# fulcrumgenomics/fgumi

Hardware: AMD Instinct MI355X
Metric: simplex consensus throughput, input raw reads/s (depth-8 x 150bp) (higher is better)
Workload: dtype f64

## Files before the change

fgumi_amd/csrc/api.cpp:

```cpp
#include <chrono>
#include <cstdio>
#include <stdexcept>
#include <cstring>
#include <mutex>
#include <map>
#include <mutex>
#include <string>
#include <thread>
#include "engine.h"
#include <gnu/libc-version.h>
#include <cmath>
#include "fastpath.h"
#include "host_common.h"
#include "simgen.h"
#include "canon_core.h"
#include "reject_core.h"
#include "aln_tags_core.h"

namespace fgx {
using canon::CANON_KIND_DUPLEX; using canon::CANON_KIND_CODEC; using canon::CANON_KIND_SIMPLEX;
uint32_t launch_canon_molecules(hipStream_t s, int kind, const canon::Params& P, const canon::CodecParams& PC, const uint8_t* d_blob,
                                const uint64_t* d_rec_off, const uint32_t* d_rec_len, const uint32_t* d_grp_first, const uint32_t* d_def, uint32_t nd,
                                const uint64_t* d_first, uint8_t* d_out, const uint64_t* d_out_off, uint32_t* d_out_len, int* d_status,
                                canon::Delta* d_delta, DevBuf& slabs, canon::RefRuns* d_runs, const rej::Params* PS);
// ... 1357 lines not shown
uint32_t fgx_debug_last_duplex_deep(const fgx_caller* c) { return (c && c->fast) ? c->fast->fp.last_duplex_deep : 0u; }
uint32_t fgx_debug_last_duplex_deep_capped(const fgx_caller* c) { return (c && c->fast) ? c->fast->fp.last_duplex_deep_capped : 0u; }
uint32_t fgx_debug_last_codec_deep(const fgx_caller* c) { return (c && c->fast) ? c->fast->fp.last_codec_deep : 0u; }
uint32_t fgx_debug_last_codec_deep_capped(const fgx_caller* c) { return (c && c->fast) ? c->fast->fp.last_codec_deep_capped : 0u; }
uint32_t fgx_debug_last_boundary_rounds(const fgx_caller* c) { return c ? c->last_boundary_rounds : 0u; }
void fgx_debug_last_split_builds(const fgx_caller* c, uint64_t* out4) {
  if (!out4) return;
  out4[0] = out4[1] = out4[2] = out4[3] = 0;
  if (c && c->fast) { const FastPath& f = c->fast->fp; out4[0] = f.last_packed_families; out4[1] = f.last_classic_families; out4[2] = f.last_split_build; out4[3] = f.last_first_stage_retries; }
}
void fgx_debug_split_first_slice(double mean_records, int packed, uint32_t* out4) {
  if (!out4) return;
  out4[0] = s2_first_slice_bytes(mean_records, packed != 0);
  out4[1] = out4[0] - s2_tile_bytes(mean_records);
  out4[2] = (uint32_t)sizeof(FullItem);
  out4[3] = S2_FLAG_DESC_BYTES;
}
void fgx_debug_last_packed_rows(const fgx_caller* c, uint64_t* out2) {
  if (!out2) return;
  out2[0] = out2[1] = 0;
  if (c && c->fast) { out2[0] = c->fast->fp.last_packed_clean; out2[1] = c->fast->fp.last_packed_general; }
}
void fgx_debug_last_packed_overlap(const fgx_caller* c, uint64_t* out3) {
  if (!out3) return;
  for (int i = 0; i < 3; i++) out3[i] = (c && c->fast) ? c->fast->fp.last_packed_overlap[i] : 0;
}
void fgx_debug_last_full_results(const fgx_caller* c, uint64_t* out4) {
  if (!out4) return;
  for (int i = 0; i < 4; i++) out4[i] = (c && c->fast) ? c->fast->fp.last_full_results[i] : 0;
}
uint64_t fgx_debug_last_full_results_over(const fgx_caller* c) { return (c && c->fast) ? c->fast->fp.last_full_results[4] : 0; }
int fgx_debug_full_range_whole(uint32_t base, uint32_t items, uint32_t cap) { return full_range_whole(base, items, cap) ? 1 : 0; }
void fgx_debug_last_chain(const fgx_caller* c, uint32_t* out2) { if (out2) { out2[0] = (c && c->fast) ? c->fast->fp.last_launches : 0u; out2[1] = (c && c->fast) ? c->fast->fp.last_host_syncs : 0u; } }
uint32_t fgx_debug_last_routed(const fgx_caller* c) { return (c && c->fast) ? c->fast->fp.last_routed : 0u; }
int fgx_debug_last_direct(const fgx_caller* c) { return (c && c->fast) ? c->fast->fp.last_direct : 0; }
void fgx_set_general_only(fgx_caller* c, int on) { if (c) c->general_only = on != 0; }
void fgx_set_fast_lds_bytes(fgx_caller* c, uint32_t bytes) { if (c) { if (!c->fast) c->fast = new FastState(); c->fast->fp.lds_tile_bytes_large = bytes; } }

int fgx_call_columns(fgx_caller* c, const uint8_t* bases, const uint8_t* quals, uint32_t n_cols, uint32_t depth, uint8_t* out_base,
                     uint8_t* out_qual, uint32_t* out_depth, uint32_t* out_errors) {
  if (!c) return 1;
  c->err.clear();
  try {
    ColumnBatch& B = c->batch;
    B.clear();
    std::vector<uint8_t> rb, rq;
    for (uint32_t j0 = 0; j0 < n_cols; j0 += 4096) {
      uint32_t w = std::min<uint32_t>(4096, n_cols - j0);
      uint32_t rd0 = (uint32_t)B.reads.size();
      for (uint32_t i = 0; i < depth; i++) {
        rb.resize(w); rq.resize(w);
        for (uint32_t k = 0; k < w; k++) { rb[k] = bases[(size_t)(j0 + k) * depth + i]; rq[k] = quals[(size_t)(j0 + k) * depth + i]; }
        B.add_read(rb.data(), rq.data(), w);
      }
      if (depth == 0) { B.add_job(rd0, 0, w); continue; }
      if (depth == 1) { rb.assign(w, 'N'); rq.assign(w, 0); B.add_read(rb.data(), rq.data(), w); B.add_job(rd0, 2, w); }
      else B.add_job(rd0, depth, w);
    }
    ColParams prm{0, 0};
    c->run_columns(B, prm);
    for (uint32_t j = 0; j < n_cols; j++) { out_base[j] = B.ob[j]; out_qual[j] = B.oq[j]; out_depth[j] = B.od[j]; out_errors[j] = B.oe[j]; }
    return 0;
  } catch (const std::exception& ex) { c->err = ex.what(); return 3; }
}

int fgx_device_libm(fgx_caller* c, int op, const double* x, double* y, uint64_t n) {
// ... 118 lines not shown
```

fgumi_amd/csrc/fastpath.hip:

```cpp
#if !defined(FGX_WAVEMU)
#include <hipcub/hipcub.hpp>
#endif
#include "bamrec.h"
#include "canon_core.h"
#include "engine.h"
#include <cstdlib>
#include <memory>
#include <string>
#include <type_traits>
#include "fastpath.h"
#include "gate_core.h"
#include "packed_core.h"
#include "record_core.h"

#if defined(FGX_WAVEMU)
#define FGX_DYN_LDS(name) uint8_t* const name = wavemu::dyn_lds()
#define FGX_PIN(...) ((void)0)
#define FGX_UNDEF4(a, b, c, d) do { a = 0; b = 0; c = 0; d = 0; } while (0)
#define FGX_MEM_PIN() ((void)0)
#define FGX_CONST_AS
#else
#define FGX_DYN_LDS(name) extern __shared__ __align__(16) uint8_t name[]
#define FGX_PIN(...) asm volatile("" : __VA_ARGS__)
#define FGX_UNDEF4(a, b, c, d) asm volatile("" : "=v"(a), "=v"(b), "=v"(c), "=v"(d))
// ... 2487 lines not shown
    const double ll[4] = {sLL[k][0], sLL[k][1], sLL[k][2], sLL[k][3]};
    const uint32_t ob = sObs[k];
    const bool is_rx = (dest >> 63) != 0;
    const ConsensusTables& T = is_rx ? P.TU->t : P.T->t;
    int bi;
    uint8_t q;
    call_full(T, ll, &bi, &q);
    if (is_rx) {
      const uint64_t d = dest & ~(1ull << 63);
      P.rx_base[(size_t)(d >> 8) * P.rx_stride + (d & 0xFF)] = bi >= 0 ? "ACGT"[bi] : 'N';
    } else finish(dest, bi, q, ob & 0xFF, (ob >> 8) & 0xFF, (ob >> 16) & 0xFF, ob >> 24, (sKind[k] >> 31) != 0, sSlot[k]);
  }
  if (P.stats) {
    const uint32_t t_arr = wave_sum(n_arr), t_scat = wave_sum(n_scat);
    if ((threadIdx.x & 63) == 0) {
      unsigned long long* fs = P.stats + (size_t)((blockIdx.x * 4 + blockIdx.y + (threadIdx.x >> 6)) & (STAT_SLOTS - 1)) * FULL_STATS_STRIDE;
      if (t_arr) atomicAdd(&fs[0], (unsigned long long)t_arr);
      if (t_scat) atomicAdd(&fs[1], (unsigned long long)t_scat);
    }
  }
}

#include "record_writers.inc"

#include "simplex_wave2.inc"
#include "simplex_seg.inc"
#include "simplex_split.inc"
#include "simplex_deep.inc"
#include "duplex_deep.inc"
#include "codec_deep.inc"
#include "simplex_wide.inc"
#include "duplex_meth.inc"

__global__ void k_col_bound(const uint32_t* __restrict__ grp_first, const uint32_t* __restrict__ rec_len, const uint64_t* __restrict__ rec_off, uint32_t n_grp,
                            uint64_t* __restrict__ bound, uint32_t max_ends, uint4* __restrict__ fam_desc, unsigned long long* __restrict__ small_recs, uint64_t* __restrict__ sizes_tail) {
  uint32_t g = blockIdx.x * blockDim.x + threadIdx.x;
  {
    uint32_t mine = 0;
    if (g < n_grp) { const uint32_t n = grp_first[g + 1] - grp_first[g]; mine = (grp_first[g + 1] >= grp_first[g] && n <= 64u) ? n : 0u; }
    __shared__ unsigned int s_tot;
    if (threadIdx.x == 0) s_tot = 0;
    __syncthreads();
    const uint32_t tot = wave_sum(mine);
    if ((threadIdx.x & 63) == 0 && tot) atomicAdd(&s_tot, tot);
    __syncthreads();
    if (threadIdx.x == 0 && s_tot) atomicAdd(small_recs, (unsigned long long)s_tot);
  }
  if (g >= n_grp) return;
  if (g == n_grp - 1) { bound[n_grp] = 0; *sizes_tail = 0; }
  uint32_t a = grp_first[g], b = grp_first[g + 1], mx = 0;
  {
    uint32_t r = a;
    if (((uintptr_t)rec_len & 15u) == 0) {
      for (; r < b && (r & 3u); r++) { const uint32_t l = rec_len[r]; mx = l > mx ? l : mx; }
      for (; r + 4 <= b; r += 4) {
        const uint4 v = *(const uint4*)(rec_len + r);
        const uint32_t m01 = v.x > v.y ? v.x : v.y, m23 = v.z > v.w ? v.z : v.w, m4 = m01 > m23 ? m01 : m23;
        mx = m4 > mx ? m4 : mx;
      }
    }
    for (; r < b; r++) { const uint32_t l = rec_len[r]; mx = l > mx ? l : mx; }
  }
  uint32_t lb = mx > 33 ? (mx - 33) * 2 / 3 + 1 : 1;
  uint32_t ends = (b - a) < max_ends ? (b - a) : max_ends;
  bound[g] = (uint64_t)ends * lb + COL_BOUND_PAD;
  uint64_t lo = 0;
  uint32_t span = 0xFFFFFFFFu;
  if (b > a) {
    lo = rec_off[a];
    const uint64_t hi = rec_off[b - 1] + rec_len[b - 1];
    if (hi >= lo && hi - lo < 0xFFFFFFFFull) span = (uint32_t)(hi - lo);
  }
  fam_desc[g] = make_uint4((uint32_t)lo, (uint32_t)(lo >> 32), span, b - a);
}

__global__ void k_reduce_stats(const unsigned long long* __restrict__ slots, unsigned long long* __restrict__ out, const unsigned long long* __restrict__ full_stats, uint32_t full_out) {
  uint32_t k = threadIdx.x;
  if (k >= 32 && k < 32 + FULL_STATS_N + OV_STATS_N) {
    unsigned long long v = 0;
    for (int i = 0; i < STAT_SLOTS; i++) v += full_stats[(size_t)i * FULL_STATS_STRIDE + (k - 32)];
    out[full_out + (k - 32)] = v;
  }
  if (k >= 32) return;
  unsigned long long v = 0;
  for (int i = 0; i < STAT_SLOTS; i++) v += slots[(size_t)i * 32 + k];
  out[k < FGX_STATS_LEN ? k : 40 + (k - FGX_STATS_LEN)] = v;
}

}

#define FGX_SYNC(st) do { fp.last_host_syncs++; hip_check(hipStreamSynchronize(st), "sync"); } while (0)
#define FGX_LAUNCH(kernel, grid, block, lds, st, ...) do { fp.last_launches++; hipLaunchKernelGGL((kernel), grid, block, lds, st, __VA_ARGS__); hip_check(hipGetLastError(), #kernel " launch"); } while (0)

void FastPath::release() {
  for (DevBuf* b : {&d_ends, &d_sizes, &d_offsets, &d_code, &d_qual, &d_depth, &d_err, &d_misc, &d_deferred, &d_out, &d_scan_tmp, &d_strings, &d_obs, &d_obs_all, &d_retry2,
                    &d_retry, &d_bound, &d_colbase, &d_statslots, &d_full_items, &d_full_count, &d_full_res, &d_full_flag, &d_retry_old, &d_w2img, &d_famdesc, &d_fwimg,
                    &d_split_rec, &d_split_fam, &d_split_out, &d_route, &d_s2img, &d_dir_size, &d_dir_off, &d_dir_base, &d_slot_desc, &d_slot_err, &d_out2, &d_scan_tmp2, &d_big, &d_deep_sizes, &d_deep_row0, &d_deep_rows, &d_deep_walk, &d_deep_fams, &d_deep_out, &d_deep_out2, &d_wide_scratch, &d_wide_pass, &d_wide_pass0, &d_wide_depth, &d_mflag, &d_mu, &d_mt, &d_mslot, &d_mcontigs})
    b->free_();
  for (int i = 0; i < 4; i++) if (ev[i]) { (void)hipEventDestroy(ev[i]); ev[i] = nullptr; }
  if (s2) {
    (void)hipStreamDestroy(s2); s2 = nullptr;
    for (int i = 0; i < MAX_CHUNKS; i++) { if (ev_chunk[i]) { (void)hipEventDestroy(ev_chunk[i]); ev_chunk[i] = nullptr; } if (ev_cols[i]) { (void)hipEventDestroy(ev_cols[i]); ev_cols[i] = nullptr; } }
    if (ev_fin) { (void)hipEventDestroy(ev_fin); ev_fin = nullptr; }
    if (ev_sample) { (void)hipEventDestroy(ev_sample); ev_sample = nullptr; }
  }
}
// ... 172 lines not shown
  void next_list(uint32_t n) { cur_list = lists[out_list]; n_cur = n; out_list ^= 1; }

  void set_up() {
    fp.last_meth_device = 0; fp.last_meth_clipped = 0; fp.last_direct = 0; fp.last_split_chunks = 0;
    if (!fp.canon_second_pass) fp.last_deep_clipped = fp.last_duplex_deep = fp.last_duplex_deep_capped = fp.last_codec_deep = fp.last_codec_deep_capped = 0;
    fp.last_routed = 0; fp.last_big_families = 0; fp.last_deep_families = 0; fp.last_wide_families = 0; fp.last_packed_families = 0; fp.last_classic_families = 0; fp.last_packed_clean = 0; fp.last_packed_general = 0; for (uint64_t& v : fp.last_packed_overlap) v = 0; for (uint64_t& v : fp.last_full_results) v = 0; fp.last_split_build = 0; fp.last_first_stage_retries = 0;
    fp.d_ends.reserve((size_t)n_slots * (duplex ? sizeof(DuplexDesc) : codec ? sizeof(CodecDesc) : sizeof(EndDesc)));
    fp.d_sizes.reserve(((size_t)n_slots + 1) * 8);
    fp.d_offsets.reserve(((size_t)n_slots + 1) * 8);
    fp.d_deferred.reserve((size_t)n_grp * 4);
    fp.d_misc.reserve(MISC_WORDS * 8);
    hip_check(hipMemsetAsync(fp.d_misc.p, 0, MISC_WORDS * 8, s), "memset");
    misc = fp.d_misc.as<unsigned long long>();
    const std::string strs = c->prefix + c->rg;
    fp.d_strings.reserve(strs.size() + 16);
    if (!strs.empty()) hip_check(hipMemcpyAsync(fp.d_strings.p, strs.data(), strs.size(), hipMemcpyHostToDevice, s), "H2D strings");
    for (int i = 0; i < 4; i++) if (!fp.ev[i]) hip_check(hipEventCreate(&fp.ev[i]), "hipEventCreate");
    fp.d_bound.reserve(((size_t)n_grp + 1) * 8); fp.d_colbase.reserve(((size_t)n_grp + 1) * 8);
    fp.d_statslots.reserve((size_t)STAT_SLOTS * 32 * 8);
    hip_check(hipMemsetAsync(fp.d_statslots.p, 0, (size_t)STAT_SLOTS * 32 * 8, s), "memset");
    fp.d_famdesc.reserve((size_t)n_grp * 16);
    hip_check(hipEventRecord(c->ev0, s), "event");
    hip_check(hipEventRecord(fp.ev[0], s), "event");
    fpw = mean_recs >= 1.0 ? (uint32_t)(64.0 / mean_recs) : 16u;
    fpw = fpw < 1u ? 1u : fpw > 16u ? 16u : fpw;
    if (sw.split_fpw) fpw = sw.split_fpw;
    n_chunks = ps.chunks >= 1 ? (uint32_t)ps.chunks : std::min<uint32_t>(8u, std::max<uint32_t>(1u, n_grp / 150000u));
    if (n_chunks > (uint32_t)FastPath::MAX_CHUNKS - 1) n_chunks = FastPath::MAX_CHUNKS - 1;
    chunk_fam_raw = (n_grp + n_chunks - 1) / n_chunks;
    chunk_fam = ((chunk_fam_raw + 4 * fpw - 1) / (4 * fpw)) * (4 * fpw);
  }

  void bound_columns() {
    FGX_LAUNCH(k_col_bound, dim3((n_grp + 1023) / 1024), dim3(1024), 0, s, d_grp_first, d_rec_len, d_rec_off, n_grp, fp.d_bound.as<uint64_t>(), duplex ? 4u : codec ? 2u : 3u,
               fp.d_famdesc.as<uint4>(), misc + MISC_SMALL_RECS, fp.d_sizes.as<uint64_t>() + n_slots);
    scan_u64(fp.d_bound.as<uint64_t>(), fp.d_colbase.as<uint64_t>(), n_grp + 1, "scan bound");
    uint64_t col_total = 0;
    hip_check(hipMemcpyAsync(&col_total, fp.d_colbase.as<uint64_t>() + n_grp, 8, hipMemcpyDeviceToHost, s), "D2H");
    unsigned long long small_recs = 0;
    hip_check(hipMemcpyAsync(&small_recs, misc + MISC_SMALL_RECS, 8, hipMemcpyDeviceToHost, s), "D2H");
    sync();
    use_split = simplex_v2 && sw.split && !seg4 && (sw.split_mode == 2 || (double)small_recs >= 0.5 * (double)n_rec);
    direct = use_split && sw.direct && !fp.direct_off && !meth_dev;
    if (early_parse && !use_split) join_s2(fp.ev_chunk[0]);
    col_cap = col_total + 64;
    if (direct) {
      dir_cap = std::max<uint64_t>(col_cap * 6 + (uint64_t)n_slots * 64 + 4096, fp.dir_cap_min);
      fp.d_out.reserve(dir_cap + 64);
      fp.d_dir_size.reserve((size_t)n_grp * 4 + 64); fp.d_dir_off.reserve((size_t)n_grp * 8 + 64); fp.d_dir_base.reserve((FastPath::MAX_CHUNKS + 2) * 8);
      fp.d_slot_desc.reserve((size_t)n_slots * sizeof(SlotDesc)); fp.d_slot_err.reserve((size_t)n_slots * 4);
      hip_check(hipMemsetAsync(fp.d_dir_size.p, 0, (size_t)n_grp * 4, s), "memset");
      hip_check(hipMemsetAsync(fp.d_dir_base.p, 0, (FastPath::MAX_CHUNKS + 2) * 8, s), "memset");
      hip_check(hipMemsetAsync(fp.d_slot_err.p, 0, (size_t)n_slots * 4, s), "memset");
      hip_check(hipMemsetAsync(fp.d_sizes.p, 0, ((size_t)n_slots + 1) * 8, s), "memset");
    }
    fp.d_code.reserve(col_cap + 64); fp.d_qual.reserve(col_cap + 64); fp.d_err.reserve(col_cap * 2 + 64);
    if (meth_dev || meth_dup) {
      fp.d_mflag.reserve(col_cap + 64); fp.d_mu.reserve(col_cap * 2 + 64); fp.d_mt.reserve(col_cap * 2 + 64);
      fp.d_mslot.reserve((size_t)n_slots * (meth_dup ? sizeof(DuplexMethSlot) : sizeof(MethSlot)) + 64);
    }
    if (duplex) fp.d_obs.reserve(col_cap * 4); else fp.d_depth.reserve(col_cap * 2 + 64);
    if (dup_cap) fp.d_obs_all.reserve(col_cap * 4);
  }

  void fill_params() {
    memset(&P, 0, sizeof(P));
    P.blob = d_blob; P.rec_off = d_rec_off; P.rec_len = d_rec_len; P.grp_first = d_grp_first;
// ... 747 lines not shown
```

fgumi_amd/csrc/simplex_split.inc:

```

#ifndef FGX_S2_OCC
#define FGX_S2_OCC 6
#endif
#ifndef FGX_S2_OCC_PACKED
#define FGX_S2_OCC_PACKED 7
#endif
#ifndef FGX_S2_PAIRS
#define FGX_S2_PAIRS 256
#endif

#ifndef FGX_S2_F32
#define FGX_S2_F32 1
#endif
#ifndef FGX_S2_FMASEL
#define FGX_S2_FMASEL 1
#endif
#ifndef FGX_S2_NOSUM
#define FGX_S2_NOSUM 1
#endif
#ifndef FGX_S2_PREGATE
#define FGX_S2_PREGATE 1
#endif
struct S2Lds {
  GateTables g;
// ... 10 lines not shown
  struct { uint32_t cap; } g;
  uint8_t t1[96];
};
struct S2Head {
  GateTables g;
  uint8_t t1[96];
  alignas(16) float pairf[FGX_S2_PAIRS][2];
};
constexpr uint32_t S2_HEAD_BYTES = (uint32_t)(offsetof(S2Lds, pair));
static_assert(sizeof(S2Head) == S2_HEAD_BYTES, "S2Head is the head of S2Lds");
static_assert(S2_HEAD_BYTES % 16 == 0, "the head of S2Lds is copied in 16-byte pieces");
static_assert(sizeof(S2Lds) % 16 == 0, "S2Lds is copied in 16-byte pieces");
inline void build_s2_image(S2Image& I, const ConsensusTables& t) {
  memset(&I, 0, sizeof(I));
  S2Lds& L = I.lds;
  fill_gate_tables(L.g, t);
  for (uint32_t i = 0; i < FGX_S2_PAIRS; i++) {
    const uint32_t q = i < 93 ? i : 93;
    L.pair[i][0] = t.correct[q]; L.pair[i][1] = t.error_per_alt[q];
  }
  fill_pairs_f32(L.pairf, FGX_S2_PAIRS, t);
  pk::fill_t1(L.t1, t);
  pk::fill_t2(I.t2, t);
}

#if defined(FGX_WAVEMU)
__device__ __forceinline__ uint32_t s2_mul24(uint32_t a, uint32_t b) { return (a & 0xFFFFFFu) * (b & 0xFFFFFFu); }
#else
__device__ __forceinline__ uint32_t s2_mul24(uint32_t a, uint32_t b) { uint32_t r; asm("v_mul_u32_u24_e32 %0, %1, %2" : "=v"(r) : "v"(a), "v"(b)); return r; }
#endif
__device__ __forceinline__ uint32_t mbcnt64(unsigned long long m) { return __builtin_amdgcn_mbcnt_hi((uint32_t)(m >> 32), __builtin_amdgcn_mbcnt_lo((uint32_t)m, 0u)); }

constexpr uint32_t SP_HEAD = 48, SP_AUX = 64, SP_LANE = SP_HEAD + SP_AUX;
constexpr uint32_t SP_WAVE_LDS = 64 * SP_LANE + 16;
template <class AfterRound>
__device__ __forceinline__ void s2_parse_wave(const FastParams& P, const uint32_t g0, const uint32_t nf, uint8_t* const Wv, const uint8_t* const sTagCls,
                                              uint64_t* __restrict__ bound, const uint32_t max_ends, uint4* __restrict__ fam_desc, AfterRound&& after_round) {
  typedef uint32_t u32x4 __attribute__((ext_vector_type(4)));
  const uint32_t lane = threadIdx.x & 63;
  uint8_t* const Wh = Wv + lane * SP_LANE;
  uint8_t* const Wa = Wh + SP_HEAD;
  const uint32_t gf = P.grp_first[g0 + (lane < nf ? lane : nf)];
  const unsigned long long below = (1ull << lane) - 1ull;
  SplitRec* const out_rec = P.split_rec;
  SplitFam* const out_fam = P.split_fam;

  uint32_t fa = 0;
  while (fa < nf) {
    const uint32_t ra = rlane(gf, fa);
    uint32_t fb = fa + 1;
    while (fb < nf) {
      const uint32_t nx = rlane(gf, fb + 1), cur = rlane(gf, fb);
      if (nx < cur || nx - ra > 64u) break;
      fb++;
    }
    const uint32_t rb = rlane(gf, fb);
    const uint32_t nrec = rb >= ra ? rb - ra : 0u;
    if (nrec > 64u) {
      const uint32_t g = g0 + fa;
      uint32_t mx = 0;
      for (uint32_t i = lane; i < nrec; i += 64) { const uint32_t l = P.rec_len[ra + i]; mx = l > mx ? l : mx; }
      mx = uni(wave_max(mx));
      if (lane == 0) {
        const uint32_t lb = mx > 33 ? (mx - 33) * 2 / 3 + 1 : 1;
        const uint32_t ends = nrec < max_ends ? nrec : max_ends;
        if (bound) {
          bound[g] = (uint64_t)ends * lb + COL_BOUND_PAD;
// ... 54 lines not shown
#pragma unroll
      for (uint32_t u = 0; u < SP_AUX / 16; u++) *(u32x4*)(Wa + 16 * u) = ap[u];
    }
    wave_sync();
    if (parse) {
      ref_id = unm ? unmapped_ref_key(lane) : H.ref_id; pos = H.pos;
      if (record::streaming_flags_odd(H, true)) odd = true;
      if (!unm && !record::single_block_op(ld32u(Wh, l_name), l_seq)) odd = true;
      AuxTags ax;
      if (aux_in_lds) aux_walk(Wa, sTagCls, 0u, aux_len, P, ax);
      else aux_walk(rec + aux_rel, sTagCls, 0u, aux_len, P, ax);
      if (ax.oddw) odd = true;
      const record::TagFields tg = record::unpack_tags(ax);
      has_mi = tg.has_mi; mi_rel = aux_rel + tg.mi_lo; mi_len = tg.mi_len;
      has_rx = tg.has_rx; rx_rel = aux_rel + tg.rx_lo; rx_len = tg.rx_len;
      has_cb = tg.has_cb; cb_rel = aux_rel + tg.cb_lo; cb_len = tg.cb_len;
      if (!odd && tg.has_mc && !(flags & (bam::F_UNMAPPED | bam::F_MATE_UNMAPPED))) {
        const uint32_t ML = record::mc_single_m(tg.mc_len, [&]() { return aux_in_lds ? ld64u(Wa, tg.mc_lo) : gld64(rec + aux_rel + tg.mc_lo); });
        if (ML == 0 || !record::mate_in_range(M)) odd = true;
        else clip = record::single_m_mate_clip(H, ref_id, M, (int32_t)ML);
      }
      if (!odd) hash = record::name_hash30(name_len, [&](uint32_t o) { return ld32u(Wh, o); }, [&](uint32_t o) { return ld64u(Wh, o); });
    }
    if (act && sl == 0 && !odd && record::first_record_odd(has_mi, mi_len, P.prefix_len)) odd = true;
    if (act && !odd && (mi_len > 255 || rx_len > 255 || cb_len > 255)) odd = true;
    const bool rev = (flags & bam::F_REVERSE) != 0;
    const uint32_t ty = (!act || odd) ? 0u : (flags & bam::F_FIRST) ? 1u : (flags & bam::F_LAST) ? 2u : 0u;
    const uint32_t cls = ty == 2u ? 1u : 0u;
    const uint32_t off_lo = (uint32_t)off, off_hi = (uint32_t)(off >> 32);
    const unsigned long long off0 = (unsigned long long)fbc(off_lo, 0) | ((unsigned long long)fbc(off_hi, 0) << 32);
    if (act && !odd && (off < off0 || off - off0 > 0x7FFF0000ull)) odd = true;

    const uint32_t kh = (hash << 2) | ty;
    const uint32_t inf = l_seq | (cls << 16) | ((rev ? 1u : 0u) << 17);
    const uint32_t nmax = uni(wave_max(n));
    int cmate = -1, clater = -1;
    uint32_t max_a = cls == 0u ? l_seq : 0u, max_b = cls == 1u ? l_seq : 0u, max_len = len;
    bool irregular = false;
    for (uint32_t k = 1; k < nmax; k++) {
      const uint32_t up = sl + k;
      const bool wrap = up >= n, inrange = k < n;
      const uint32_t s = wrap ? up - n : up;
      const uint32_t src = seg_lo + (inrange ? s : sl);
      const uint32_t okh = (uint32_t)__shfl((int)kh, (int)src), oinf = (uint32_t)__shfl((int)inf, (int)src), olen = (uint32_t)__shfl((int)len, (int)src);
      const uint32_t d = okh ^ kh;
      const int as_later = (d == 0 && !wrap && inrange) ? (int)s : -1;
      const int as_mate = (d == 3 && inrange) ? (int)s : -1;
      clater = as_later > clater ? as_later : clater;
      cmate = as_mate > cmate ? as_mate : cmate;
      const uint32_t ol = oinf & 0xFFFF, ocls = (oinf >> 16) & 1u, orev = (oinf >> 17) & 1u;
      if (inrange) {
        if (ocls == 0u) max_a = ol > max_a ? ol : max_a; else max_b = ol > max_b ? ol : max_b;
        max_len = olen > max_len ? olen : max_len;
        if (ocls == cls && (orev != (rev ? 1u : 0u) || (rev && ol != l_seq))) irregular = true;
      }
    }
    if (ty != 1u || !P.overlap) { cmate = -1; clater = -1; }
    int mate = -1;
    bool collide = false;
    {
      const int other = clater >= 0 ? clater : cmate;
      const uint32_t osl = other >= 0 ? (uint32_t)other : sl;
      const uint32_t onl = fbc(name_len, osl);
      if (other >= 0) {
        bool same = onl == name_len;
        const uint8_t* const Wo = Wv + (seg_lo + osl) * SP_LANE;
        for (uint32_t i = 0; i < name_len && same; i += 8) {
          unsigned long long wa = ld64u(Wo, i), wb = ld64u(Wh, i);
          if (i + 8 > name_len) { const unsigned long long mk = (1ULL << (8 * (name_len - i))) - 1; wa &= mk; wb &= mk; }
          if (wa != wb) same = false;
        }
        if (!same) collide = true;
        else if (clater < 0) mate = cmate;
      }
    }
    const uint32_t msrc = mate >= 0 ? (uint32_t)mate : sl;
    const int32_t pos_b = (int32_t)fbc((uint32_t)pos, msrc), ref_b = (int32_t)fbc((uint32_t)ref_id, msrc);
    const uint32_t len_b = fbc(l_seq, msrc);
    uint32_t ov_cnt = 0, ov_off1 = 0, ov_off2 = 0;
    if (mate >= 0 && ref_id == ref_b) {
      const int32_t s1 = pos + 1, e1 = pos + (int32_t)l_seq, s2 = pos_b + 1, e2 = pos_b + (int32_t)len_b;
      const int32_t lox = s1 > s2 ? s1 : s2, hix = e1 < e2 ? e1 : e2;
      if (hix >= lox) { ov_cnt = (uint32_t)(hix - lox + 1); ov_off1 = (uint32_t)(lox - s1); ov_off2 = (uint32_t)(lox - s2); }
    }
    bool ov_uniform;
    {
      const unsigned long long ovm = fbal(act && ov_cnt != 0);
      const uint32_t fp = ovm ? (uint32_t)__builtin_ctzll(ovm) : 0u;
      const uint32_t key = ov_cnt | (ov_off1 << 16);
      const uint32_t k0 = fbc(key, fp), k1 = fbc(ov_off2, fp);
      const unsigned long long other_geometry = fbal(act && ov_cnt != 0 && (key != k0 || ov_off2 != k1));
      ov_uniform = ovm != 0 && other_geometry == 0;
    }
    const unsigned long long in_a = fbal(act && cls == 0u), in_b = fbal(act && cls == 1u);
    const uint32_t m_a = (uint32_t)__popcll(in_a), m_b = (uint32_t)__popcll(in_b);
    const unsigned long long mine_below = (cls ? in_b : in_a) & ((1ull << sl) - 1ull);
    const uint32_t slot = (uint32_t)__popcll(mine_below) + (cls ? m_a : 0u);
    const uint32_t mate_slot = fbc(slot, msrc);
    const unsigned long long with_rx = fbal(act && has_rx);
    const uint32_t rx0_rel = fbc(rx_rel, 0), rx0_len = fbc(rx_len, 0);
    const uint32_t rx0_win = fbc((aux_in_lds ? 1u : 0u) | (aux_rel << 1), 0);
    bool rx_diff = false;
    if (act && !odd && has_rx && sl != 0) {
      if (rx_len != rx0_len) rx_diff = true;
      else if (aux_in_lds && (rx0_win & 1u)) {
        const uint8_t* const W0 = Wv + seg_lo * SP_LANE + SP_HEAD;
        const uint32_t o0 = rx0_rel - (rx0_win >> 1), o1 = rx_rel - aux_rel;
        for (uint32_t i = 0; i < rx_len && !rx_diff; i += 8) {
          unsigned long long wa = ld64u(W0, o0 + i), wb = ld64u(Wa, o1 + i);
          if (i + 8 > rx_len) { const unsigned long long mk = (1ULL << (8 * (rx_len - i))) - 1; wa &= mk; wb &= mk; }
          if (wa != wb) rx_diff = true;
        }
      } else {
        const uint8_t* const r0p = P.blob + off0 + rx0_rel;
        const uint8_t* const rp = rec + rx_rel;
        for (uint32_t i = 0; i < rx_len && !rx_diff; i += 8) {
          unsigned long long wa = gld64(r0p + i), wb = gld64(rp + i);
          if (i + 8 > rx_len) { const unsigned long long mk = (1ULL << (8 * (rx_len - i))) - 1; wa &= mk; wb &= mk; }
          if (wa != wb) rx_diff = true;
        }
      }
    }
    const bool f_odd = fbal(odd) != 0, f_coll = fbal(collide) != 0, f_irr = fbal(irregular) != 0, f_rxd = fbal(rx_diff) != 0;
    const bool f_frag = fbal(act && ty == 0u) != 0, f_pair = fbal(act && ty != 0u) != 0;
    const bool f_mix = mixed_unmapped_end(act, flags, fbal);
    const bool rx_all = with_rx == nmask, rx_none = with_rx == 0;
    const uint32_t maxl = max_a > max_b ? max_a : max_b;
    const uint32_t qs = maxl <= 160u ? 160u : (maxl + 15u) & ~15u, ss = maxl <= 160u ? 80u : ((maxl + 1u) / 2u + 15u) & ~15u;
    const uint32_t qc = qs >> 4, sc = ss >> 4;
    const uint32_t need = n * (qs + ss);
    bool take = !f_odd && !f_coll && !f_irr && !f_rxd && !f_mix && !(f_frag && f_pair) && (rx_all || rx_none) && n >= 1u && maxl >= 1u;
    if (rx_all && rx0_len > (uint32_t)FAST_RX_CAP) take = false;
    if (P.max_reads >= 0 && ((long long)m_a > P.max_reads || (long long)m_b > P.max_reads)) take = false;
    if (need > 60000u || maxl > 4000u) take = false;
    if (P.dir_size && (m_a > 16u || m_b > 16u)) take = false;

    if (P.dir_size) {
      uint8_t* const Wm = Wv;
      Wm[lane] = 0;
      wave_sync();
      if (act && mate >= 0) Wm[seg_lo + (uint32_t)mate] = (uint8_t)(sl + 1u);
      wave_sync();
      const uint32_t pm = Wm[lane];
      const int partner = mate >= 0 ? mate : (int)pm - 1;
      const uint32_t psl = partner >= 0 ? (uint32_t)partner : sl;
      const uint32_t p_cnt = fbc(ov_cnt, psl), p_o1 = fbc(ov_off1, psl), p_o2 = fbc(ov_off2, psl);
      const uint32_t p_seq = fbc(seq_rel, psl), p_lseq = fbc(l_seq, psl), p_lo = fbc(off_lo, psl), p_hi = fbc(off_hi, psl);
      uint32_t wo = 0, mo = 0, wc = 0;
      if (partner >= 0) { if (mate >= 0) { wo = ov_off1; mo = ov_off2; wc = ov_cnt; } else { wo = p_o2; mo = p_o1; wc = p_cnt; } }
      uint32_t fin = 0;
      if (act && take) {
        const uint8_t* const prec = P.blob + (((unsigned long long)p_hi << 32) | p_lo);
        const uint32_t qrel = seq_rel + ((l_seq + 1u) >> 1), pqrel = p_seq + ((p_lseq + 1u) >> 1);
        const uint32_t min_bq = P.min_input_bq & 0xFFu;
        uint32_t flr = l_seq > clip ? l_seq - clip : 0u;
        while (flr > 0) {
// ... 52 lines not shown
      auto rec_bytes = [&](uint32_t Lc, uint32_t fk, uint32_t kept_n) -> uint32_t {
        const bool hcb = P.cell0 && fbc(has_cb ? 1u : 0u, fk) != 0;
        const uint32_t cbl = fbc(cb_len, fk);
        const uint32_t nm = P.prefix_len + 1u + mi0;
        return 4u + 32u + nm + 1u + (Lc + 1u) / 2u + Lc + (3u + P.rg_len + 1u) + 4u + 4u + 7u + (P.per_base_tags ? 2u * (8u + 2u * Lc) : 0u) +
               (3u + mi0 + 1u) + (hcb ? 3u + cbl + 1u : 0u) + ((rx_all && kept_n) ? 3u + rx0_len + 1u : 0u);
      };
      const uint32_t sz_f = rec_bytes(clen[0], fk_e[0], rem_e[0]), sz_1 = rec_bytes(clen[1], fk_e[1], rem_e[1]), sz_2 = rec_bytes(clen[2], fk_e[2], rem_e[2]);
      const uint32_t dsize = !take ? 0u : has_frag ? sz_f : has_pair ? sz_1 + sz_2 : 0u;
      if (act && sl == 0) P.dir_size[g] = dsize;
    }

    if (act) {
      SplitRec R;
      R.body_off = (uint32_t)(off - off0);
      R.seq_rel = (uint16_t)seq_rel; R.l_seq = (uint16_t)l_seq; R.clip = (uint16_t)clip;
      R.ov_off1 = (uint16_t)ov_off1; R.ov_off2 = (uint16_t)ov_off2; R.ov_cnt = (uint16_t)ov_cnt;
      R.slot = (uint8_t)slot; R.mate_slot = (uint8_t)mate_slot;
      R.bits = (uint8_t)(ty | ((rev ? 1u : 0u) << 2) | ((has_cb ? 1u : 0u) << 3));
      R.cb_len = (uint8_t)cb_len; R.cb_rel = (uint16_t)cb_rel; R.mi_rel = (uint16_t)mi_rel;
      R.mi_len = (uint8_t)mi_len; R.rx_len = (uint8_t)rx_len; R.rx_rel = (uint16_t)rx_rel;
      R._pad = 0;
      out_rec[r] = R;
    }
    if (bound && act && sl == 0) {
      const uint32_t lb = max_len > 33 ? (max_len - 33) * 2 / 3 + 1 : 1;
      const uint32_t ends = n < max_ends ? n : max_ends;
      bound[g] = (uint64_t)ends * lb + COL_BOUND_PAD;
    }
    {
      const uint32_t last = n ? n - 1 : 0;
      const unsigned long long end = off + len;
      const unsigned long long hi = (unsigned long long)fbc((uint32_t)end, last) | ((unsigned long long)fbc((uint32_t)(end >> 32), last) << 32);
      const uint32_t fa_l = in_a ? (uint32_t)__builtin_ctzll(in_a) : 0u, fb_l = in_b ? (uint32_t)__builtin_ctzll(in_b) : 0u;
      const uint32_t ra_v = fbc(rev ? 1u : 0u, fa_l), rb_v = fbc(rev ? 1u : 0u, fb_l);
      if (act && sl == 0) {
        const uint32_t span = (hi >= off && hi - off < 0xFFFFFFFFull) ? (uint32_t)(hi - off) : 0xFFFFFFFFu;
        if (bound) fam_desc[g] = make_uint4((uint32_t)off, (uint32_t)(off >> 32), span, n);
        SplitFam F;
        F.flags = take ? 1u : 0u;
        F.need_bytes = need;
        F.qs = (uint16_t)qs; F.ss = (uint16_t)ss;
        F.n = (uint8_t)n; F.m_a = (uint8_t)m_a; F.m_b = (uint8_t)m_b; F.type_a = (uint8_t)((f_frag ? 0u : 1u) | (ov_uniform ? 2u : 0u));
        F.rev_a = (uint8_t)(in_a ? ra_v : 0u); F.rev_b = (uint8_t)(in_b ? rb_v : 0u);
        F.rx_len = (uint8_t)(rx_all ? rx0_len : 0u); F.rx_all = (uint8_t)(rx_all ? 1u : 0u);
        F.len_a = (uint16_t)(max_a < 65535u ? max_a : 65535u); F.len_b = (uint16_t)(max_b < 65535u ? max_b : 65535u);
        const uint32_t cpr = qc + sc;
        F.inv_cpr = cpr ? (16777216u + cpr - 1u) / cpr : 0u;
        F.qc = (uint16_t)qc; F.sc = (uint16_t)sc;
        out_fam[g] = F;
      }
    }
    {
      const uint32_t fj = fa + lane;
      const uint32_t a0 = (uint32_t)__shfl((int)gf, (int)(fj < nf ? fj : nf)), a1 = (uint32_t)__shfl((int)gf, (int)(fj + 1 <= nf ? fj + 1 : nf));
      if (fj < fb && a1 <= a0) {
        const uint32_t ge = g0 + fj;
        if (bound) { bound[ge] = 0; fam_desc[ge] = make_uint4(0u, 0u, 0xFFFFFFFFu, a1 == a0 ? 0u : a1 - a0); }
        SplitFam F;
        memset(&F, 0, sizeof(F));
        out_fam[ge] = F;
      }
    }
    }
    after_round(fa, fb);
    fa = fb;
  }
// ... 37 lines not shown
    const s2_f32x2 w_sel2 = {w_sel, w_sel}; \
    acc2 = __builtin_elementwise_fma((pr_), w_sel2, acc2);    \
    cntf += w_sel; \
  } while (0)
#else
#define S2_OBSERVE(q_, sb_, pr_) do { \
    const uint32_t w_q = (q_), w_c = ((uint32_t)(sb_) >> ish) & 15u; \
    const unsigned long long qm = __builtin_amdgcn_uicmp(w_q, min_bq, 35 ); \
    const unsigned long long bm = __builtin_amdgcn_uicmp(__builtin_amdgcn_ubfe(allow, w_c, 1u), 0u, 33 ); \
    suspect |= qm & ~bm; \
    if (__builtin_amdgcn_inverse_ballot_w64(qm & bm)) { allow = 1u << w_c; n1++; S2_ADD(pr_); } \
  } while (0)
#endif
#if FGX_S2_F32
#define S2_ADD(pr_) do { acc2 += (pr_); } while (0)
#else
#define S2_ADD(pr_) do { kahan2(s1, c1, (pr_).x); kahan2(sR, cR, (pr_).y); } while (0)
#endif
#if FGX_S2_F32
typedef float s2_f32x2 __attribute__((ext_vector_type(2)));
#define S2_PAIR(pr_, q_) s2_f32x2 pr_ = *(const s2_f32x2*)(pairs + ((q_) << 3))
#else
#define S2_PAIR(pr_, q_) double2 pr_ = *(const double2*)(pairs + S2_PAIR_OFF(q_))
#endif
#define S2_PIN4(a_, b_, c_, d_) FGX_PIN("+v"(a_.x), "+v"(a_.y), "+v"(b_.x), "+v"(b_.y), "+v"(c_.x), "+v"(c_.y), "+v"(d_.x), "+v"(d_.y))
#define S2_PIN1(a_) FGX_PIN("+v"(a_.x), "+v"(a_.y))
#define S2_OBSERVE_FAST(q_, sb_) do { \
    const uint32_t w_c = __builtin_amdgcn_ubfe((uint32_t)(sb_), ish, 4u); \
    const bool w_g = (uint32_t)(q_) >= min_bq; \
    const uint32_t w_t = w_g ? w_c : 0u; \
    f_or |= w_t; f_sum += w_t; f_cnt += w_g ? 1u : 0u; \
  } while (0)

typedef unsigned short s2_u16x2 __attribute__((ext_vector_type(2)));
__device__ __forceinline__ uint32_t s2_pkmax(uint32_t a, uint32_t b) { s2_u16x2 x, y; __builtin_memcpy(&x, &a, 4); __builtin_memcpy(&y, &b, 4); x = __builtin_elementwise_max(x, y); uint32_t r; __builtin_memcpy(&r, &x, 4); return r; }
__device__ __forceinline__ uint32_t s2_pkmin(uint32_t a, uint32_t b) { s2_u16x2 x, y; __builtin_memcpy(&x, &a, 4); __builtin_memcpy(&y, &b, 4); x = __builtin_elementwise_min(x, y); uint32_t r; __builtin_memcpy(&r, &x, 4); return r; }
__device__ __forceinline__ void s2_st16(uint8_t* p, uint32_t v) { const uint16_t w = (uint16_t)v; __builtin_memcpy(p, &w, 2); }
struct S2DirRec { uint32_t base, Lc, type, fk, kept, o_seq, o_qual, o_rg, o_t3, o_cd, o_ce, o_mi, o_cb, o_rx, size, hcb, cbl; };

__device__ uint32_t g_s2_dbg[64];
constexpr uint32_t S2_PACKED_MAX_ROWS = 31;
__device__ __forceinline__ bool s2_packed_shape(uint32_t m_a, uint32_t m_b, uint32_t len_a, uint32_t len_b, uint32_t nsafe) {
  const bool oa = m_a < 2u || (m_a >= nsafe && m_a <= S2_PACKED_MAX_ROWS), ob = m_b < 2u || (m_b >= nsafe && m_b <= S2_PACKED_MAX_ROWS);
  return oa && ob && ((len_a + 7u) >> 3) + ((len_b + 7u) >> 3) <= 64u;
}

constexpr uint32_t S2_PAD_FRONT = 8;
__host__ __device__ __forceinline__ uint32_t s2_padded_b(uint32_t lc_a) { return S2_PAD_FRONT + ((lc_a + 7u) & ~7u) + 16u; }
static_assert(COL_BOUND_PAD >= S2_PAD_FRONT + 7 + 16 + 7 + 8, "the column bound's padding covers the packed build's layout: 8 + r8(lc_a) + 16 + r8(lc_b) + 8 <= 2 lc + 2 + COL_BOUND_PAD");
template <int COLS> struct S2SharedOf {
#if FGX_S2_F32
  typedef typename std::conditional<COLS == 1, S2Tiny, S2Head>::type type;
#else
  typedef S2Lds type;
#endif
};
typedef uint32_t s2_u32x4 __attribute__((ext_vector_type(4)));
template <bool AGAIN> struct S2Args { static __device__ __forceinline__ const FastParams& of(const FastParams& P) { return P; } };
#if !defined(FGX_WAVEMU)
template <> struct S2Args<true> {
  static __device__ __forceinline__ const FGX_CONST_AS FastParams& of(const FastParams&) {
    const FGX_CONST_AS FastParams* k = (const FGX_CONST_AS FastParams*)__builtin_amdgcn_kernarg_segment_ptr();
    FGX_PIN("+s"(k));
    return *k;
  }
};
#endif
template <int QS_T, int SS_T, int DIRECT, int COLS, bool FUSED>
// ... 1110 lines not shown
```

Measured before the change: 3.244 billion.

## Rework column-bound kernel into grid-stride wave tiles and vectorize split-parse pairing

The column-bound kernel changes from one thread per family walking its own records to a grid-stride loop over 64-family wave tiles. Each tile reads record lengths cooperatively and does a segmented max reduction through LDS and bpermute. In the simplex split parser, the per-family O(n) shuffle loop for mate/later matching now scans keys staged in LDS four at a time. The max length and irregular-orientation checks now use a log-step packed max and ballots instead. The aim is to remove serialized, divergent per-thread walks, at the cost of more LDS traffic and extra wave syncs.

```diff
diff --git a/fgumi_amd/csrc/api.cpp b/fgumi_amd/csrc/api.cpp
--- a/fgumi_amd/csrc/api.cpp
+++ b/fgumi_amd/csrc/api.cpp
@@ -1413,6 +1413,13 @@
 uint64_t fgx_debug_last_full_results_over(const fgx_caller* c) { return (c && c->fast) ? c->fast->fp.last_full_results[4] : 0; }
 int fgx_debug_full_range_whole(uint32_t base, uint32_t items, uint32_t cap) { return full_range_whole(base, items, cap) ? 1 : 0; }
 void fgx_debug_last_chain(const fgx_caller* c, uint32_t* out2) { if (out2) { out2[0] = (c && c->fast) ? c->fast->fp.last_launches : 0u; out2[1] = (c && c->fast) ? c->fast->fp.last_host_syncs : 0u; } }
+int fgx_debug_last_col_bound(const fgx_caller* c, uint64_t* bound, uint32_t* desc4, uint32_t n) {
+  if (!c || !c->fast || !bound || !desc4) return 0;
+  const FastPath& f = c->fast->fp;
+  if (!f.d_bound.p || !f.d_famdesc.p || f.d_bound.cap < ((size_t)n + 1) * 8 || f.d_famdesc.cap < (size_t)n * 16) return 0;
+  if (hipDeviceSynchronize() != hipSuccess || hipMemcpy(bound, f.d_bound.p, ((size_t)n + 1) * 8, hipMemcpyDeviceToHost) != hipSuccess) return 0;
+  return hipMemcpy(desc4, f.d_famdesc.p, (size_t)n * 16, hipMemcpyDeviceToHost) == hipSuccess ? 1 : 0;
+}
 uint32_t fgx_debug_last_routed(const fgx_caller* c) { return (c && c->fast) ? c->fast->fp.last_routed : 0u; }
 int fgx_debug_last_direct(const fgx_caller* c) { return (c && c->fast) ? c->fast->fp.last_direct : 0; }
 void fgx_set_general_only(fgx_caller* c, int on) { if (c) c->general_only = on != 0; }
diff --git a/fgumi_amd/csrc/fastpath.hip b/fgumi_amd/csrc/fastpath.hip
--- a/fgumi_amd/csrc/fastpath.hip
+++ b/fgumi_amd/csrc/fastpath.hip
@@ -2543,46 +2543,99 @@
 #include "simplex_wide.inc"
 #include "duplex_meth.inc"
 
-__global__ void k_col_bound(const uint32_t* __restrict__ grp_first, const uint32_t* __restrict__ rec_len, const uint64_t* __restrict__ rec_off, uint32_t n_grp,
+#ifndef FGX_COL_BOUND_FORM
+#define FGX_COL_BOUND_FORM 0
+#endif
+#ifndef FGX_COL_BOUND_NO_ATOMIC
+#define FGX_COL_BOUND_NO_ATOMIC 0
+#endif
+constexpr uint32_t COL_BOUND_WAVES = 4, COL_BOUND_MAX_BLOCKS = 2048;
+__device__ __forceinline__ uint32_t col_bound_walk(const uint32_t* __restrict__ rec_len, uint32_t a, uint32_t b) {
+  uint32_t r = a, mx = 0;
+  if (((uintptr_t)rec_len & 15u) == 0) {
+    for (; r < b && (r & 3u); r++) { const uint32_t l = rec_len[r]; mx = l > mx ? l : mx; }
+    for (; r + 4 <= b; r += 4) {
+      const uint4 v = *(const uint4*)(rec_len + r);
+      const uint32_t m01 = v.x > v.y ? v.x : v.y, m23 = v.z > v.w ? v.z : v.w, m4 = m01 > m23 ? m01 : m23;
+      mx = m4 > mx ? m4 : mx;
+    }
+  }
+  for (; r < b; r++) { const uint32_t l = rec_len[r]; mx = l > mx ? l : mx; }
+  return mx;
+}
+__global__ __launch_bounds__(64 * COL_BOUND_WAVES) void k_col_bound(const uint32_t* __restrict__ grp_first, const uint32_t* __restrict__ rec_len, const uint64_t* __restrict__ rec_off, uint32_t n_grp,
                             uint64_t* __restrict__ bound, uint32_t max_ends, uint4* __restrict__ fam_desc, unsigned long long* __restrict__ small_recs, uint64_t* __restrict__ sizes_tail) {
-  uint32_t g = blockIdx.x * blockDim.x + threadIdx.x;
-  {
-    uint32_t mine = 0;
-    if (g < n_grp) { const uint32_t n = grp_first[g + 1] - grp_first[g]; mine = (grp_first[g + 1] >= grp_first[g] && n <= 64u) ? n : 0u; }
-    __shared__ unsigned int s_tot;
-    if (threadIdx.x == 0) s_tot = 0;
-    __syncthreads();
-    const uint32_t tot = wave_sum(mine);
-    if ((threadIdx.x & 63) == 0 && tot) atomicAdd(&s_tot, tot);
-    __syncthreads();
-    if (threadIdx.x == 0 && s_tot) atomicAdd(small_recs, (unsigned long long)s_tot);
-  }
-  if (g >= n_grp) return;
-  if (g == n_grp - 1) { bound[n_grp] = 0; *sizes_tail = 0; }
-  uint32_t a = grp_first[g], b = grp_first[g + 1], mx = 0;
-  {
-    uint32_t r = a;
-    if (((uintptr_t)rec_len & 15u) == 0) {
-      for (; r < b && (r & 3u); r++) { const uint32_t l = rec_len[r]; mx = l > mx ? l : mx; }
-      for (; r + 4 <= b; r += 4) {
-        const uint4 v = *(const uint4*)(rec_len + r);
-        const uint32_t m01 = v.x > v.y ? v.x : v.y, m23 = v.z > v.w ? v.z : v.w, m4 = m01 > m23 ? m01 : m23;
-        mx = m4 > mx ? m4 : mx;
-      }
-    }
-    for (; r < b; r++) { const uint32_t l = rec_len[r]; mx = l > mx ? l : mx; }
-  }
-  uint32_t lb = mx > 33 ? (mx - 33) * 2 / 3 + 1 : 1;
-  uint32_t ends = (b - a) < max_ends ? (b - a) : max_ends;
-  bound[g] = (uint64_t)ends * lb + COL_BOUND_PAD;
-  uint64_t lo = 0;
-  uint32_t span = 0xFFFFFFFFu;
-  if (b > a) {
-    lo = rec_off[a];
-    const uint64_t hi = rec_off[b - 1] + rec_len[b - 1];
-    if (hi >= lo && hi - lo < 0xFFFFFFFFull) span = (uint32_t)(hi - lo);
-  }
-  fam_desc[g] = make_uint4((uint32_t)lo, (uint32_t)(lo >> 32), span, b - a);
+  __shared__ uint32_t s_first[COL_BOUND_WAVES][64], s_max[COL_BOUND_WAVES][64];
+  __shared__ unsigned int s_tot;
+  const uint32_t lane = threadIdx.x & 63, wv = threadIdx.x >> 6;
+  if (threadIdx.x == 0) s_tot = 0;
+  __syncthreads();
+  const uint32_t n_tiles = (n_grp + 63u) >> 6, tile_step = gridDim.x * COL_BOUND_WAVES;
+  uint32_t mine = 0;
+#if FGX_COL_BOUND_FORM == 1
+  for (uint32_t tile = blockIdx.x * COL_BOUND_WAVES + wv; tile < n_tiles; tile += tile_step) {
+    const uint32_t g = tile * 64u + lane;
+    if (g >= n_grp) continue;
+    const uint32_t a = grp_first[g], b = grp_first[g + 1];
+    mine += (b >= a && b - a <= 64u) ? b - a : 0u;
+    uint64_t lo = 0, hi = 0;
+    if (b > a) { lo = rec_off[a]; hi = rec_off[b - 1] + rec_len[b - 1]; }
+    const uint32_t mx = col_bound_walk(rec_len, a, b);
+#else
+  for (uint32_t tile = uni(blockIdx.x * COL_BOUND_WAVES + wv); tile < n_tiles; tile += tile_step) {
+    const uint32_t g0 = tile * 64u, nf = n_grp - g0 < 64u ? n_grp - g0 : 64u;
+    const uint32_t g = g0 + lane;
+    const bool fam = lane < nf;
+    const uint32_t a = grp_first[g0 + (fam ? lane : nf)], b = grp_first[g0 + (fam ? lane + 1u : nf)];
+    mine += (b >= a && b - a <= 64u) ? b - a : 0u;
+    uint64_t lo = 0, hi = 0;
+    if (b > a) { lo = rec_off[a]; hi = rec_off[b - 1] + rec_len[b - 1]; }
+    s_first[wv][lane] = a;
+    s_max[wv][lane] = 0;
+    wave_sync();
+    const uint32_t r0 = rlane(a, 0), r1 = uni(wave_max(b));
+    uint32_t mx;
+    if (__ballot(b < a) != 0) mx = col_bound_walk(rec_len, a, b);
+    else {
+      for (uint32_t rb = r0; rb < r1; rb += 64u) {
+        const uint32_t r = rb + lane;
+        const bool in = r1 - rb > lane;
+        const uint32_t len = in ? rec_len[r] : 0u;
+        uint32_t f = 0;
+#pragma unroll
+        for (uint32_t st = 32; st > 0; st >>= 1) f += s_first[wv][f + st] <= r ? st : 0u;
+        const uint32_t f_prev = (uint32_t)__builtin_amdgcn_ds_bpermute((int)((lane - 1u) << 2), (int)f);
+        const unsigned long long heads = __ballot(lane == 0 || f_prev != f) >> 1;
+        const unsigned long long ahead = heads >> lane;
+        const uint32_t room = ahead ? (uint32_t)__builtin_ctzll(ahead) : 63u - lane;
+        uint32_t m = len;
+#pragma unroll
+        for (uint32_t d = 1; d < 64; d <<= 1) {
+          const uint32_t o = (uint32_t)__builtin_amdgcn_ds_bpermute((int)((lane + d) << 2), (int)m);
+          m = (d <= room && o > m) ? o : m;
+        }
+        if (in && (lane == 0 || f_prev != f)) atomicMax(&s_max[wv][f], m);
+      }
+      wave_sync();
+      mx = s_max[wv][lane];
+    }
+    wave_sync();
+    if (!fam) continue;
+#endif
+    if (g == n_grp - 1) { bound[n_grp] = 0; *sizes_tail = 0; }
+    const uint32_t lb = mx > 33 ? (mx - 33) * 2 / 3 + 1 : 1;
+    const uint32_t ends = (b - a) < max_ends ? (b - a) : max_ends;
+    bound[g] = (uint64_t)ends * lb + COL_BOUND_PAD;
+    uint32_t span = 0xFFFFFFFFu;
+    if (b > a && hi >= lo && hi - lo < 0xFFFFFFFFull) span = (uint32_t)(hi - lo);
+    fam_desc[g] = make_uint4((uint32_t)lo, (uint32_t)(lo >> 32), span, b - a);
+  }
+  const uint32_t tot = wave_sum(mine);
+  if (lane == 0 && tot) atomicAdd(&s_tot, tot);
+  __syncthreads();
+#if !FGX_COL_BOUND_NO_ATOMIC
+  if (threadIdx.x == 0 && s_tot) atomicAdd(small_recs, (unsigned long long)s_tot);
+#endif
 }
 
 __global__ void k_reduce_stats(const unsigned long long* __restrict__ slots, unsigned long long* __restrict__ out, const unsigned long long* __restrict__ full_stats, uint32_t full_out) {
@@ -2821,7 +2874,8 @@
   }
 
   void bound_columns() {
-    FGX_LAUNCH(k_col_bound, dim3((n_grp + 1023) / 1024), dim3(1024), 0, s, d_grp_first, d_rec_len, d_rec_off, n_grp, fp.d_bound.as<uint64_t>(), duplex ? 4u : codec ? 2u : 3u,
+    const uint32_t cb_blocks = std::min<uint32_t>(COL_BOUND_MAX_BLOCKS, std::max<uint32_t>(1u, (n_grp + 64u * COL_BOUND_WAVES - 1u) / (64u * COL_BOUND_WAVES)));
+    FGX_LAUNCH(k_col_bound, dim3(cb_blocks), dim3(64 * COL_BOUND_WAVES), 0, s, d_grp_first, d_rec_len, d_rec_off, n_grp, fp.d_bound.as<uint64_t>(), duplex ? 4u : codec ? 2u : 3u,
                fp.d_famdesc.as<uint4>(), misc + MISC_SMALL_RECS, fp.d_sizes.as<uint64_t>() + n_slots);
     scan_u64(fp.d_bound.as<uint64_t>(), fp.d_colbase.as<uint64_t>(), n_grp + 1, "scan bound");
     uint64_t col_total = 0;
diff --git a/fgumi_amd/csrc/simplex_split.inc b/fgumi_amd/csrc/simplex_split.inc
--- a/fgumi_amd/csrc/simplex_split.inc
+++ b/fgumi_amd/csrc/simplex_split.inc
@@ -66,7 +66,11 @@
 __device__ __forceinline__ uint32_t mbcnt64(unsigned long long m) { return __builtin_amdgcn_mbcnt_hi((uint32_t)(m >> 32), __builtin_amdgcn_mbcnt_lo((uint32_t)m, 0u)); }
 
 constexpr uint32_t SP_HEAD = 48, SP_AUX = 64, SP_LANE = SP_HEAD + SP_AUX;
-constexpr uint32_t SP_WAVE_LDS = 64 * SP_LANE + 16;
+constexpr uint32_t SP_KEYS = 64 * SP_LANE + 16;
+constexpr uint32_t SP_WAVE_LDS = SP_KEYS + 64 * 4;
+static_assert(SP_KEYS % 16 == 0, "the pairing loop reads four keys per LDS instruction");
+typedef unsigned short s2_u16x2 __attribute__((ext_vector_type(2)));
+__device__ __forceinline__ uint32_t s2_pkmax(uint32_t a, uint32_t b) { s2_u16x2 x, y; __builtin_memcpy(&x, &a, 4); __builtin_memcpy(&y, &b, 4); x = __builtin_elementwise_max(x, y); uint32_t r; __builtin_memcpy(&r, &x, 4); return r; }
 template <class AfterRound>
 __device__ __forceinline__ void s2_parse_wave(const FastParams& P, const uint32_t g0, const uint32_t nf, uint8_t* const Wv, const uint8_t* const sTagCls,
                                               uint64_t* __restrict__ bound, const uint32_t max_ends, uint4* __restrict__ fam_desc, AfterRound&& after_round) {
@@ -187,30 +191,53 @@
     if (act && !odd && (off < off0 || off - off0 > 0x7FFF0000ull)) odd = true;
 
     const uint32_t kh = (hash << 2) | ty;
-    const uint32_t inf = l_seq | (cls << 16) | ((rev ? 1u : 0u) << 17);
     const uint32_t nmax = uni(wave_max(n));
     int cmate = -1, clater = -1;
-    uint32_t max_a = cls == 0u ? l_seq : 0u, max_b = cls == 1u ? l_seq : 0u, max_len = len;
-    bool irregular = false;
-    for (uint32_t k = 1; k < nmax; k++) {
-      const uint32_t up = sl + k;
-      const bool wrap = up >= n, inrange = k < n;
-      const uint32_t s = wrap ? up - n : up;
-      const uint32_t src = seg_lo + (inrange ? s : sl);
-      const uint32_t okh = (uint32_t)__shfl((int)kh, (int)src), oinf = (uint32_t)__shfl((int)inf, (int)src), olen = (uint32_t)__shfl((int)len, (int)src);
-      const uint32_t d = okh ^ kh;
-      const int as_later = (d == 0 && !wrap && inrange) ? (int)s : -1;
-      const int as_mate = (d == 3 && inrange) ? (int)s : -1;
-      clater = as_later > clater ? as_later : clater;
-      cmate = as_mate > cmate ? as_mate : cmate;
-      const uint32_t ol = oinf & 0xFFFF, ocls = (oinf >> 16) & 1u, orev = (oinf >> 17) & 1u;
-      if (inrange) {
-        if (ocls == 0u) max_a = ol > max_a ? ol : max_a; else max_b = ol > max_b ? ol : max_b;
-        max_len = olen > max_len ? olen : max_len;
-        if (ocls == cls && (orev != (rev ? 1u : 0u) || (rev && ol != l_seq))) irregular = true;
-      }
+    {
+      uint8_t* const Kr = Wv + SP_KEYS;
+      *(uint32_t*)(Kr + 4u * lane) = kh;
+      wave_sync();
+      const uint32_t kspan = uni(wave_max((seg_lo & 3u) + n));
+      uint32_t ka = (seg_lo & ~3u) << 2, s = 0u - (seg_lo & 3u);
+#pragma unroll 1
+      for (uint32_t k = 0; k < kspan; k += 4) {
+        const u32x4 ok = *(const u32x4*)(Kr + (ka & 255u));
+#define S2_KEY(okh_, j_) do { \
+          const uint32_t d = (okh_) ^ kh, sj = s + (j_); \
+          cmate = (d == 3u && sj < n) ? (int)sj : cmate;     \
+          clater = (d == 0u && sj < n) ? (int)sj : clater;   \
+        } while (0)
+        S2_KEY(ok.x, 0u); S2_KEY(ok.y, 1u); S2_KEY(ok.z, 2u); S2_KEY(ok.w, 3u);
+#undef S2_KEY
+        ka += 16u; s += 4u;
+      }
+      clater = clater > (int)sl ? clater : -1;
     }
     if (ty != 1u || !P.overlap) { cmate = -1; clater = -1; }
+    const unsigned long long in_a = fbal(act && cls == 0u), in_b = fbal(act && cls == 1u);
+    const uint32_t fa_l = in_a ? (uint32_t)__builtin_ctzll(in_a) : 0u, fb_l = in_b ? (uint32_t)__builtin_ctzll(in_b) : 0u;
+    bool f_irr;
+    {
+      const unsigned long long rv = fbal(act && rev);
+      const uint32_t l0a = fbc(l_seq, fa_l), l0b = fbc(l_seq, fb_l);
+      const unsigned long long ldiff = fbal(act && l_seq != (cls ? l0b : l0a));
+      const unsigned long long rv_a = rv & in_a, rv_b = rv & in_b;
+      f_irr = (((rv_a ^ in_a) | (ldiff & in_a)) != 0) & (rv_a != 0) | (((rv_b ^ in_b) | (ldiff & in_b)) != 0) & (rv_b != 0);
+    }
+    uint32_t max_ab = (sl == 0u && l_seq > 0xFFFFu) ? 0u : (l_seq & 0xFFFFu) << (((cls | (l_seq >> 16)) & 1u) << 4);
+    uint32_t max_len = len;
+    for (uint32_t d = 1; d < nmax; d <<= 1) {
+      const uint32_t oab = (uint32_t)__builtin_amdgcn_ds_bpermute((int)((lane + d) << 2), (int)max_ab);
+      const bool mine = sl + d < n;
+      max_ab = s2_pkmax(max_ab, mine ? oab : 0u);
+      if (bound) {
+        const uint32_t olen = (uint32_t)__builtin_amdgcn_ds_bpermute((int)((lane + d) << 2), (int)max_len);
+        max_len = (mine && olen > max_len) ? olen : max_len;
+      }
+    }
+    const uint32_t f_ab = fbc(max_ab, 0);
+    const uint32_t own_a = cls == 0u ? l_seq : 0u, own_b = cls == 1u ? l_seq : 0u;
+    const uint32_t max_a = (f_ab & 0xFFFFu) > own_a ? (f_ab & 0xFFFFu) : own_a, max_b = (f_ab >> 16) > own_b ? (f_ab >> 16) : own_b;
     int mate = -1;
     bool collide = false;
     {
@@ -247,7 +274,6 @@
       const unsigned long long other_geometry = fbal(act && ov_cnt != 0 && (key != k0 || ov_off2 != k1));
       ov_uniform = ovm != 0 && other_geometry == 0;
     }
-    const unsigned long long in_a = fbal(act && cls == 0u), in_b = fbal(act && cls == 1u);
     const uint32_t m_a = (uint32_t)__popcll(in_a), m_b = (uint32_t)__popcll(in_b);
     const unsigned long long mine_below = (cls ? in_b : in_a) & ((1ull << sl) - 1ull);
     const uint32_t slot = (uint32_t)__popcll(mine_below) + (cls ? m_a : 0u);
@@ -276,7 +302,7 @@
         }
       }
     }
-    const bool f_odd = fbal(odd) != 0, f_coll = fbal(collide) != 0, f_irr = fbal(irregular) != 0, f_rxd = fbal(rx_diff) != 0;
+    const bool f_odd = fbal(odd) != 0, f_coll = fbal(collide) != 0, f_rxd = fbal(rx_diff) != 0;
     const bool f_frag = fbal(act && ty == 0u) != 0, f_pair = fbal(act && ty != 0u) != 0;
     const bool f_mix = mixed_unmapped_end(act, flags, fbal);
     const bool rx_all = with_rx == nmask, rx_none = with_rx == 0;
@@ -395,7 +421,6 @@
       const uint32_t last = n ? n - 1 : 0;
       const unsigned long long end = off + len;
       const unsigned long long hi = (unsigned long long)fbc((uint32_t)end, last) | ((unsigned long long)fbc((uint32_t)(end >> 32), last) << 32);
-      const uint32_t fa_l = in_a ? (uint32_t)__builtin_ctzll(in_a) : 0u, fb_l = in_b ? (uint32_t)__builtin_ctzll(in_b) : 0u;
       const uint32_t ra_v = fbc(rev ? 1u : 0u, fa_l), rb_v = fbc(rev ? 1u : 0u, fb_l);
       if (act && sl == 0) {
         const uint32_t span = (hi >= off && hi - off < 0xFFFFFFFFull) ? (uint32_t)(hi - off) : 0xFFFFFFFFu;
@@ -499,8 +524,6 @@
     f_or |= w_t; f_sum += w_t; f_cnt += w_g ? 1u : 0u; \
   } while (0)
 
-typedef unsigned short s2_u16x2 __attribute__((ext_vector_type(2)));
-__device__ __forceinline__ uint32_t s2_pkmax(uint32_t a, uint32_t b) { s2_u16x2 x, y; __builtin_memcpy(&x, &a, 4); __builtin_memcpy(&y, &b, 4); x = __builtin_elementwise_max(x, y); uint32_t r; __builtin_memcpy(&r, &x, 4); return r; }
 __device__ __forceinline__ uint32_t s2_pkmin(uint32_t a, uint32_t b) { s2_u16x2 x, y; __builtin_memcpy(&x, &a, 4); __builtin_memcpy(&y, &b, 4); x = __builtin_elementwise_min(x, y); uint32_t r; __builtin_memcpy(&r, &x, 4); return r; }
 __device__ __forceinline__ void s2_st16(uint8_t* p, uint32_t v) { const uint16_t w = (uint16_t)v; __builtin_memcpy(p, &w, 2); }
 struct S2DirRec { uint32_t base, Lc, type, fk, kept, o_seq, o_qual, o_rg, o_t3, o_cd, o_ce, o_mi, o_cb, o_rx, size, hcb, cbl; };
```

Result: slower. 3.167 billion (-2.4%).
